# wz7in/CVPR2023-VLSAT

Hardware: AMD Instinct MI355X
Metric: scenes/sec (3RScan-shaped, N=40 obj x 256 pts) (higher is better)
Workload: dtype f32

## Files before the change

cvpr2023-vlsat_amd/build.py:

```python
from __future__ import annotations

import os
import shutil
import subprocess
import sys
from concurrent.futures import ThreadPoolExecutor

HERE = os.path.dirname(os.path.abspath(__file__))
CSRC = os.path.join(HERE, "csrc")
OBJ = os.path.join(HERE, "build")
LIB = os.path.join(HERE, "libvlsat_hip.so")
SOURCES = ["engine_weights.hip", "engine_plan.hip", "engine_forward.hip", "engine_api.hip", "gemm_f32.hip", "gemm_bf16_ring.hip", "gemm_bf16_p8.hip", "gemm_splitk.hip", "flash_attn_f32.hip", "flash_attn_bf16.hip", "pointnet.hip", "pointnet_bf16.hip", "edge_gate.hip", "edge_gate_bf16.hip", "edge_gate_heads.hip", "edge_gate_bf16_heads.hip", "small_ops.hip", "stn.hip", "eval_ranks.hip", "eval_recall.hip", "scene_graph.hip", "graph_decode.hip", "prep.hip", "proximity.hip", "label_transfer.hip", "segment_merge.hip", "scene_split.hip", "calibration.hip", "mesh_segment.hip", "cloud.hip", "voxel.hip", "objects.hip", "convex.hip", "comm.hip"]
FLAGS = ["--offload-arch=gfx950", "-O3", "-std=c++17", "-fPIC", "-ffp-contract=fast", "-Wall", "-Wno-unused-function", "-Wno-unused-value", "-Wno-unused-result"]
PER_SOURCE_FLAGS = {"proximity.hip": ["-ffp-contract=off"], "label_transfer.hip": ["-ffp-contract=off"],
                    "segment_merge.hip": ["-ffp-contract=off"], "scene_split.hip": ["-ffp-contract=off"],
                    "mesh_segment.hip": ["-ffp-contract=off"], "cloud.hip": ["-ffp-contract=off"],
                    "voxel.hip": ["-ffp-contract=off"], "objects.hip": ["-ffp-contract=off"],
                    "convex.hip": ["-ffp-contract=off"]}


def _hipcc() -> str:
    exe = shutil.which("hipcc") or "/opt/rocm/bin/hipcc"
    if not os.path.exists(exe):
        raise RuntimeError("hipcc not found; the HIP library cannot be built")
    return exe


def _newest_header() -> float:
    t = 0.0
    for d in (CSRC, os.path.join(os.path.dirname(HERE), "include")):
        for f in os.listdir(d):
            if f.endswith(".h"):
                t = max(t, os.path.getmtime(os.path.join(d, f)))
    return t


EXP_LIB = os.path.join(os.path.dirname(HERE), "tools", "bin", "libvlsat_hip_exp.so")


def build(force: bool = False, verbose: bool = False, experiments: bool = False) -> str:
    obj_dir = OBJ + "_exp" if experiments else OBJ
    lib = EXP_LIB if experiments else LIB
    flags = FLAGS + (["-DVLSAT_EXPERIMENTS"] if experiments else [])
    os.makedirs(obj_dir, exist_ok=True)
    os.makedirs(os.path.dirname(lib), exist_ok=True)
    hipcc = _hipcc()
    hdr_t = _newest_header()
    jobs = []
    objs = []
    for src in SOURCES:
        s = os.path.join(CSRC, src)
        o = os.path.join(obj_dir, src.replace(".hip", ".o"))
        objs.append(o)
        if force or not os.path.exists(o) or os.path.getmtime(o) < max(os.path.getmtime(s), hdr_t):
            jobs.append([hipcc, *flags, *PER_SOURCE_FLAGS.get(src, []), "-c", s, "-o", o])

    def run(cmd):
        if verbose:
            print(" ".join(cmd), flush=True)
        r = subprocess.run(cmd, capture_output=True, text=True)
        if r.returncode:
            raise RuntimeError(f"hipcc failed: {' '.join(cmd)}\n{r.stdout}\n{r.stderr}")
        return r.stderr

    with ThreadPoolExecutor(max_workers=min(8, max(1, len(jobs)))) as ex:
# ... 11 lines not shown
```

cvpr2023-vlsat_amd/csrc/edge_gate.hip:

```cpp
#include <cstdlib>
#include "gate_core.h"
#include "gate_agg.h"

namespace vlsat {

constexpr int GT_PITCH = 68;
constexpr int GT_PITCH3 = 132;

template <bool FUSED, bool TWIN = false>
__global__ __launch_bounds__(256, 2) void edge_gate_kernel(GateArgs pa, GateArgs pb) {
    const GateArgs& p = (TWIN && blockIdx.y != 0) ? pb : pa;
    __shared__ __attribute__((aligned(16))) float sW0[128 * GT_PITCH];
    __shared__ __attribute__((aligned(16))) float sW3[32 * GT_PITCH3];
    __shared__ __attribute__((aligned(16))) char sAgg[FUSED ? 4 * AG_WAVE_BYTES : 16];
    const int tid = threadIdx.x, lane = tid & 63, wave = tid >> 6;
    const int li = lane & 31, hi = lane >> 5;

    gate_stage_f32_rows<128, 128, 64, GT_PITCH, 256>(sW0, p.w0k, tid);
    gate_stage_f32_rows<32, 32, 128, GT_PITCH3, 256>(sW3, p.w3, tid);
    float b3f[16];
#pragma unroll
    for (int r = 0; r < 16; ++r) b3f[r] = p.b3[crow32(r, hi)];
    __syncthreads();

// ... 87 lines not shown
        if (valid) grow[m] = a;
    }
    if (!valid) return;
    const float inv = 1.f / sum;
    for (int m = 0; m < dox; ++m) {
        const float pr = grow[m] * inv;
        if (p.prob) p.prob[(size_t)e * (n_heads * dox) + m * n_heads + h] = pr;
        grow[m] = pr * vrow[m];
    }
}

int launch_gate_valu(const GateArgs& a, int n_heads, int dk, int dox, hipStream_t s) {
    if (dk < 1 || dk > 128 || dox < 1) return fail(-1, "edge_gate: unsupported head geometry");
    const long rows = (long)a.n_edges * n_heads;
    hipLaunchKernelGGL(edge_gate_generic_kernel, dim3((unsigned)((rows + 63) / 64)), dim3(64), 2 * dk * 64 * sizeof(float), s, a,
                       n_heads, dk, dox);
    VLSAT_LAUNCH_CHECK("edge_gate_generic");
    return 0;
}

int launch_gate_f32(const GateArgs& a, hipStream_t s, const GateArgs* twin) {
    const int n_groups = a.row_map ? 2 * ((a.n_edges + 31) / 32) : (a.n_edges + 15) / 16;
    const int cap = a.grid_cap > 0 ? a.grid_cap : (a.agg ? 512 : 768);
    const int grid = n_groups < cap ? n_groups : cap;
    if (twin) {
        if (a.agg) hipLaunchKernelGGL((edge_gate_kernel<true, true>), dim3(grid, 2), dim3(256), 0, s, a, *twin);
        else hipLaunchKernelGGL((edge_gate_kernel<false, true>), dim3(grid, 2), dim3(256), 0, s, a, *twin);
    } else if (a.agg) hipLaunchKernelGGL((edge_gate_kernel<true, false>), dim3(grid), dim3(256), 0, s, a, a);
    else hipLaunchKernelGGL((edge_gate_kernel<false, false>), dim3(grid), dim3(256), 0, s, a, a);
    VLSAT_LAUNCH_CHECK("edge_gate");
    return 0;
}

int launch_gate(GateKernel kernel, const GateArgs& a, int n_heads, int dk, int dox, int terms, int kproj_split, hipStream_t s,
                const GateArgs* twin) {
    if (a.n_edges <= 0) return 0;
    const GateChoice can = gate_choice(kernel);
    if (a.agg && !can.fuse_agg) return fail(-1, "edge_gate: this kernel does not implement the fused aggregation");
    if (twin && !can.twin) return fail(-1, "edge_gate: this kernel does not implement a twin launch");
    if (!a.row_map && !can.row_map0) return fail(-1, "edge_gate: this kernel has the 32-edges-per-wave row map only");
    if (twin && (twin->n_edges != a.n_edges || !twin->agg != !a.agg || twin->row_map != a.row_map || twin->use_edge != a.use_edge ||
                 !twin->prob != !a.prob || twin->grid_cap != a.grid_cap || twin->src != a.src || twin->dst != a.dst))
        return fail(-1, "edge_gate: a twin launch needs two problems on the same edge list with the same options");
    if (a.agg && (!a.row_map || a.prob || (a.ld_agg & 3))) return fail(-1, "edge_gate: the fused aggregation needs the 32-edges-per-wave row map and no prob tap");
    if (kernel != GATE_VALU && ((a.ld_node & 3) || (a.gq_off & 3) || (a.v_off & 3)))
        return fail(-1, "edge_gate: ld_node/gq_off/v_off must be multiples of 4");
    if (can.bits16()) {
        if (terms != 1 && terms != 3) return fail(-1, "edge_gate_bf16: terms must be 1 or 3");
        if (kproj_split >= 2 && terms != 1) return fail(-1, "edge_gate_bf16: half-row kproj needs terms = 1");
    }
    const bool shipped = n_heads == 8 && dk == 64 && dox == 32;
    switch (kernel) {
        case GATE_VALU: return launch_gate_valu(a, n_heads, dk, dox, s);
        case GATE_F32: case GATE_16:
            if (!shipped) return fail(-1, "edge_gate: the shipped kernels are built for 8 heads x (64, 32) only");
            return kernel == GATE_F32 ? launch_gate_f32(a, s, twin) : launch_gate_16(a, terms, kproj_split, s, twin);
        case GATE_F32_HEADS: case GATE_16_HEADS:
            if (!gate_heads_built(n_heads, dk, dox) || (kernel == GATE_16_HEADS && terms == 3 && dk == 128))
                return fail(-1, "edge_gate: head geometry / terms not built on the MFMA template");
            return kernel == GATE_F32_HEADS ? launch_gate_f32_heads(a, n_heads, dk, dox, s) : launch_gate_16_heads(a, n_heads, dk, dox, terms, kproj_split, s);
    }
    return fail(-1, "edge_gate: unknown kernel");
}

}
```

cvpr2023-vlsat_amd/csrc/engine.h:

```cpp
#pragma once
#include <cstddef>
#include <cstdint>

namespace vlsat {

struct EvalScratch {
    float *obj3, *obj2, *prob3, *prob2;
    float *rel3, *rel2;
    float* sorted;
    int32_t *or3, *or2;
    int32_t *rr3, *rr2, *tr3, *tr2;
    int32_t *cn3, *cn2;
};
inline size_t eval_scratch_edge_rows(size_t E) { return E > 0 ? E : 1; }
inline size_t eval_scratch_floats(size_t N, size_t E, size_t C, size_t R) { return 5 * N * C + 2 * eval_scratch_edge_rows(E) * R; }
inline size_t eval_scratch_ints(size_t N, size_t E, size_t R) { return 2 * N + (4 * R + 2) * eval_scratch_edge_rows(E); }
inline EvalScratch eval_scratch_carve(float* f, int32_t* i, size_t N, size_t E, size_t C, size_t R) {
    const size_t Es = eval_scratch_edge_rows(E);
    EvalScratch v;
    v.obj3 = f;                v.obj2 = v.obj3 + N * C;   v.prob3 = v.obj2 + N * C;  v.prob2 = v.prob3 + N * C;
    v.rel3 = v.prob2 + N * C;  v.rel2 = v.rel3 + Es * R;  v.sorted = v.rel2 + Es * R;
    v.or3 = i;                 v.or2 = v.or3 + N;
    v.rr3 = v.or2 + N;         v.rr2 = v.rr3 + Es * R;    v.tr3 = v.rr2 + Es * R;    v.tr2 = v.tr3 + Es * R;
    v.cn3 = v.tr2 + Es * R;    v.cn2 = v.cn3 + Es;
// ... 53 lines not shown
    int D = 512, A = 256, H = 8, C_pt = 768;
    std::map<std::string, std::vector<float>> host;
    bool finalized = false;
    std::vector<float*> dev_allocs;
    std::vector<std::pair<const float*, size_t>> gemm_w;
    float *pn_w1, *pn_b1, *pn_w2, *pn_b2, *pn_w3, *pn_b3;
    float *mlp_w, *mlp_b;
    float *re_w1cat, *re_b1cat;
    float *re3_w2, *re3_b2, *re3_w3, *re3_b3, *re2_w2, *re2_b2, *re2_w3, *re2_b3;
    float *ad_w1, *ad_b1, *ad_w2h, *ad_b2h;
    vlsat::DistBiasW db{};
    std::vector<vlsat::AttnW> self_attn, cross_attn, cross_rel;
    std::vector<vlsat::GcnW> gcn3, gcn2;
    vlsat::RelHeadW rel3{}, rel2{};
    vlsat::StnW stn_obj{}, stn_re3{}, stn_re2{};
    vlsat::TripletW trip{};
    float *obj3_w, *obj3_b, *obj2_w, *obj2_b;
    bool prof = false;
    struct Rec { int cls; hipEvent_t a, b; double flops; long kernels; };
    std::vector<Rec> recs;
    Rec open[3] = {};
    bool open_ok[3] = {false, false, false};
    hipEvent_t prof_base = nullptr;
    bool prof_base_set = false;
    int prof_dual = 1;
    std::vector<hipEvent_t> ev_pool;
    size_t ev_used = 0;
    double acc_ms[vlsat::PC_COUNT] = {0};
    int64_t acc_n[vlsat::PC_COUNT] = {0};
    double acc_fl[vlsat::PC_COUNT] = {0};
    int debug_stop = -1;
    int gemm_no_dma = 0, gate_grid = 0, gate_row_map = 1, gate_heads_mfma = 1, flash_heads_bf16 = 1, gate_heads_bf16 = 1;
    int pair_twins = 1;
    int pair_max_edges = 4096;
    int gather_f16 = -1;
    int outproj_f16 = -1;
    int gemm_k_rot = -1;
    int gemm_no_p8 = 0;
    int node_attn_split = 1024;
    long config_epoch = 0;
    int gemm_p8_part_min = 0;
    int gemm_splitk_max_tiles = 64;
    int gemm_splitk = 1;
    float* sk_ws[3] = {nullptr, nullptr, nullptr};
    unsigned* sk_cnt[3] = {nullptr, nullptr, nullptr};
    int flash_bq_big_min = 4096;
    int flash_qg = 0;
    int flash_bq_big = 1;
    int flash_dma = 1;
    int gate_fuse_agg = 1;
    int flash_ablate = 0;
    int flash_pv_terms = 3;
    int flash_exact = -1;
    int gemm_small_exact = -1;
    int pointnet_exact = -1;
    int edge_pairs = 1;
    vlsat::EdgePairs pairs{};
    int gemm_exact = -1;
    int ln_resid = 1;
    int half_fmt = 1;
    int split_fmt = 1;
    int pointnet_bf16 = 1, gate_bf16 = 1;
    int flash_bf16 = 1, flash_tr = 1;
    long gemm_launches = 0;
    int cur_N = -1;
    int prec = 0, prec_edge = 0, prec_node = 0;
    int half_f16 = 0;
    int prec_attn = 0;
    std::map<const float*, std::pair<uint16_t*, uint16_t*>> split;
    std::map<const float*, uint16_t*> f16w;
    struct F16sPlanes { uint16_t *hi, *lo; int k; };
    std::map<const float*, F16sPlanes> f16s;
    std::vector<vlsat::Arena> arena_pool;
    std::vector<vlsat::Arena> arena_trash;
    std::vector<vlsat::Staging> staging;
    std::vector<hipEvent_t> spare_ev;
};

struct vlsat_plan_s {
    vlsat_ctx* h = nullptr;
    int64_t N = 0, E = 0;
    int P = 0, S = 0, max_n = 0, is_fc = 0;
    std::vector<int32_t> node_ptr;
    std::vector<int64_t> edge_ptr;
    size_t ws_bytes = 0;
    vlsat::WsParams ws;
    char* arena = nullptr;
    size_t arena_bytes = 0;
    hipEvent_t uploaded = nullptr;
    bool upload_pending = false;
    hipEvent_t last_use = nullptr;
    bool used = false;
    int32_t *d_src, *d_dst, *d_rowptr, *d_order, *d_scene_ptr;
    int32_t* d_edge_ptr32 = nullptr;
    int max_e = 0;
    int64_t* d_bias_ptr;
    int4* d_tiles;
    int n_tiles = 0;
    int4* d_tiles_big = nullptr;
    int n_tiles_big = 0;
    int fa_parts = 1;
    int4* d_krange = nullptr;
    float *fa_opart = nullptr, *fa_m = nullptr, *fa_l = nullptr;
    double flash_flops = 0;
    float *F, *X3, *X2, *NP, *QKVn, *On, *T256, *T768, *rs, *bias;
    float *H1, *H2, *E3, *E2, *Hbig, *KP, *G, *Qe, *KVe, *Oe, *R1, *R2, *prob;
// ... 38 lines not shown
```

cvpr2023-vlsat_amd/csrc/engine_api.hip:

```cpp
#include <algorithm>
#include <climits>
#include <cstdint>
#include <cstring>
#include <vector>

#include "engine.h"

using namespace vlsat;

extern "C" {

const char* vlsat_last_error(void) { return last_error_cstr(); }

int vlsat_debug_stop_after(vlsat_handle h, int32_t stage) {
    if (!h) return fail(VLSAT_EINVAL, "null handle");
    h->debug_stop = stage;
    return 0;
}

int vlsat_debug_gemm_clock_probe(int64_t* buf) {
    gemm_set_clock_probe(reinterpret_cast<long long*>(buf));
    return 0;
}

int vlsat_set_edge_attention_scope(vlsat_handle h, int32_t scope) {
    if (!h) return fail(VLSAT_EINVAL, "null handle");
    if (scope != 0 && scope != 1) return fail(VLSAT_EINVAL, "edge attention scope: 0 (per scene) or 1 (whole batch)");
    h->edge_scope = scope;
    ++h->config_epoch;
    return 0;
}

int vlsat_debug_option(vlsat_handle h, const char* name, int32_t value) {
    if (!h || !name) return fail(VLSAT_EINVAL, "vlsat_debug_option: null argument");
    const std::string k(name);
    ++h->config_epoch;
    if (k == "dual_stream") h->dual_stream = value < 0 ? 0 : value;
    else if (k == "sched") h->sched = value < 0 ? -1 : value != 0;
    else if (k == "flash_split") h->fa_split = value != 0;
    else if (k == "gemm_dma") h->gemm_no_dma = value == 0;
    else if (k == "gemm_p8") h->gemm_no_p8 = value == 0;
    else if (k == "pair_twins") h->pair_twins = value != 0;
    else if (k == "pair_max_edges") h->pair_max_edges = value < 0 ? 0 : value;
    else if (k == "gather_f16") h->gather_f16 = value < 0 ? -1 : value != 0;
    else if (k == "outproj_f16") h->outproj_f16 = value < 0 ? -1 : value != 0;
    else if (k == "gemm_k_rot") h->gemm_k_rot = value < 0 ? -1 : value > 7 ? 7 : value;
    else if (k == "gate_row_map") h->gate_row_map = value != 0;
    else if (k == "prof_dual") h->prof_dual = value != 0;
    else if (k == "gate_heads_mfma") h->gate_heads_mfma = value < 0 ? 0 : value > 2 ? 2 : value;
    else if (k == "gemm_splitk") h->gemm_splitk = value != 0;
    else if (k == "gemm_p8_part_min") h->gemm_p8_part_min = value < 0 ? 0 : value;
    else if (k == "gemm_splitk_max_tiles") h->gemm_splitk_max_tiles = value < 0 ? 0 : value;
    else if (k == "split_fmt") h->split_fmt = value != 0;
    else if (k == "ln_resid") h->ln_resid = value != 0;
    else if (k == "gate_fuse_agg") h->gate_fuse_agg = value < 0 ? 0 : value > 2 ? 2 : value;
    else if (k == "flash_pv_terms") h->flash_pv_terms = value == 2 ? 2 : 3;
    else if (k == "flash_exact") h->flash_exact = value < 0 ? -1 : value != 0;
    else if (k == "edge_pairs") h->edge_pairs = value != 0;
    else if (k == "gemm_exact") h->gemm_exact = value < 0 ? -1 : value != 0;
    else if (k == "pointnet_exact") h->pointnet_exact = value < 0 ? -1 : value != 0;
    else if (k == "gemm_small_exact") h->gemm_small_exact = value < 0 ? -1 : value != 0;
    else if (k == "flash_bf16") h->flash_bf16 = value != 0;
    else if (k == "pointnet_bf16") h->pointnet_bf16 = value != 0;
    else if (k == "gate_bf16") h->gate_bf16 = value != 0;
    else if (k == "flash_tr") h->flash_tr = value != 0;
    else if (k == "flash_bq_big") h->flash_bq_big = value != 0;
    else if (k == "flash_qg") h->flash_qg = value < 0 || value > 2 ? 0 : value;
    else if (k == "flash_bq_big_min") h->flash_bq_big_min = value < 256 ? 256 : value;
#ifdef VLSAT_EXPERIMENTS
    else if (k == "gate_grid") h->gate_grid = value > 0 ? value : 0;
    else if (k == "gate_heads_bf16") h->gate_heads_bf16 = value != 0;
    else if (k == "flash_heads_bf16") h->flash_heads_bf16 = value != 0;
    else if (k == "node_attn_split") h->node_attn_split = value;
    else if (k == "half_fmt") h->half_fmt = value != 0;
    else if (k == "flash_dma") h->flash_dma = (value == 3 || value == 4) ? value : value != 0;
    else if (k == "flash_ablate") h->flash_ablate = value;
#else
    else if (k == "gate_grid" || k == "gate_heads_bf16" || k == "flash_heads_bf16" || k == "node_attn_split" || k == "half_fmt" ||
             k == "flash_dma" || k == "flash_ablate")
        return fail(VLSAT_EINVAL, "vlsat_debug_option: " + k + " is a lab switch of the experiments build (build.py --experiments)");
#endif
    else return fail(VLSAT_EINVAL, "vlsat_debug_option: unknown option " + k);
    return 0;
}

static int test_splitk_ws(GemmArgs& a) {
    static float* ws = nullptr;
    static unsigned* cnt = nullptr;
    if (!ws) {
        VLSAT_HIP_CHECK(hipMalloc(reinterpret_cast<void**>(&ws), SPLITK_WS_FLOATS * sizeof(float)));
        VLSAT_HIP_CHECK(hipMalloc(reinterpret_cast<void**>(&cnt), SPLITK_COUNTERS * sizeof(unsigned)));
        VLSAT_HIP_CHECK(hipMemset(cnt, 0, SPLITK_COUNTERS * sizeof(unsigned)));
    }
    a.sk_ws = ws; a.sk_ws_floats = SPLITK_WS_FLOATS; a.sk_counters = cnt; a.sk_n_counters = SPLITK_COUNTERS;
    return 0;
}

int vlsat_k_gemm(const float* A, int32_t lda, const float* W, int32_t ldw, float* C, int32_t ldc, int32_t M, int32_t N,
                 int32_t K, const float* bias, const float* rowscale, const float* resid, int32_t ldr, float resid_scale,
                 const float* g0, const int32_t* gi0, int32_t ldg0, const float* g1, const int32_t* gi1, int32_t ldg1,
                 int32_t relu_a, int32_t act, void* stream) {
    GemmArgs a;
    a.A = A; a.lda = lda; a.W = W; a.ldw = ldw; a.C = C; a.ldc = ldc; a.M = M; a.N = N; a.K = K;
    a.bias = bias; a.rowscale = rowscale; a.resid = resid; a.ldr = ldr; a.resid_scale = resid_scale;
    a.g0 = g0; a.gi0 = gi0; a.ldg0 = ldg0; a.g1 = g1; a.gi1 = gi1; a.ldg1 = ldg1; a.relu_a = relu_a & 1; a.act = act;
    if (relu_a & 2) a.prefetch = 0;
    if (relu_a & 4) RUN(test_splitk_ws(a));
    if (relu_a & 8) a.no_p8 = 1;
    if (kExperiments) {
        a.force_tile = (relu_a >> 4) & 7;
// ... 516 lines not shown
    hipStream_t s = static_cast<hipStream_t>(stream);
    const size_t Es = eval_scratch_edge_rows(E);
    const EvalScratch v = eval_scratch_carve(p->ev_f, p->ev_i, N, E, C, R);
    RUN(vlsat_forward(h, p, obj_points, obj_2d_feats, descriptor, v.obj3, do2d ? v.obj2 : nullptr, v.rel3, do2d ? v.rel2 : nullptr, stream));
    GraphDecodeWs ws;
    ws.ptr = v.or3;
    ws.cnt = v.rr3;
    ws.keys = reinterpret_cast<uint32_t*>(ws.cnt + Es);
    ws.preds = reinterpret_cast<uint8_t*>(ws.keys + Es * R);
    for (int br = 0; br < (do2d ? 2 : 1); ++br) {
        float* pr = br ? v.prob2 : v.prob3;
        float* rl = br ? v.rel2 : v.rel3;
        RUN(launch_softmax_rows(br ? v.obj2 : v.obj3, C, N, C, pr, 0, s));
        if (!h->d.multi_rel_outputs) RUN(launch_exp(rl, rl, (size_t)E * R, s));
        RUN(launch_graph_decode(pr, rl, edges_e2, nullptr, p->d_scene_ptr, thresholds, N, E, C, R, n_scenes, multi_label, score_mode,
                                n_labels, max_rel, ws, br ? labels_2d : labels_3d, br ? label_probs_2d : label_probs_3d,
                                br ? rels_2d : rels_3d, br ? scores_2d : scores_3d, br ? n_valid_2d : n_valid_3d,
                                br ? n_total_2d : n_total_3d, s));
    }
    VLSAT_HIP_CHECK(hipEventRecord(p->last_use, s));
    return 0;
}

namespace {
static int scene_tables(const int64_t* node_ptr, int n_scenes, int n_heads, std::vector<int32_t>& sp, std::vector<int64_t>& bp, int* max_n) {
    if (!node_ptr || n_scenes <= 0) return fail(VLSAT_EINVAL, "bad scene table");
    sp.resize(n_scenes + 1);
    bp.resize(n_scenes);
    int64_t off = 0;
    *max_n = 0;
    for (int s = 0; s <= n_scenes; ++s) {
        if (node_ptr[s] < 0 || node_ptr[s] > INT32_MAX || (s && node_ptr[s] < node_ptr[s - 1])) return fail(VLSAT_EINVAL, "scene table must be ascending int32 offsets");
        sp[s] = (int32_t)node_ptr[s];
        if (s < n_scenes) {
            const int64_t n = node_ptr[s + 1] - node_ptr[s];
            bp[s] = off;
            off += (int64_t)n_heads * n * n;
            if (n > *max_n) *max_n = (int)n;
        }
    }
    return 0;
}
}

int vlsat_k_edge_gate(const float* kproj, const float* node, int32_t ld_node, int32_t gq_off, int32_t v_off, const int32_t* src,
                      const int32_t* dst, const float* w0k, const float* w3, const float* b3, float* gated, float* prob,
                      int32_t n_edges, int32_t n_heads, int32_t dk, int32_t dox, int32_t use_edge, int32_t variant, void* stream) {
    if (!node || !src || !dst || !w3 || !b3 || !gated || (use_edge && (!kproj || !w0k))) return fail(VLSAT_EINVAL, "edge_gate: null argument");
    if (n_edges < 0 || n_heads <= 0 || dk <= 0 || dox <= 0) return fail(VLSAT_EINVAL, "edge_gate: bad geometry");
    hipStream_t s = static_cast<hipStream_t>(stream);
    GateArgs g{};
    g.kproj = kproj; g.node = node; g.ld_node = ld_node; g.gq_off = gq_off; g.v_off = v_off; g.src = src; g.dst = dst;
    g.w0k = w0k; g.w3 = w3; g.b3 = b3; g.gated = gated; g.prob = prob; g.n_edges = n_edges; g.use_edge = use_edge != 0;
    if (variant < 0 || variant > 4) return fail(VLSAT_EINVAL, "edge_gate: variant 0..4");
    const int terms = variant == 3 ? 3 : variant == 4 ? 1 : 0;
    const GateChoice gc = variant == 1 ? gate_choice(GATE_VALU) : gate_select(n_heads, dk, dox, terms, true, variant == 2 ? 2 : 1, true);
    if (variant == 2 && gc.kernel != GATE_F32_HEADS) return fail(VLSAT_EINVAL, "edge_gate: head geometry not built on the MFMA template");
    if (terms && !gc.bits16()) return fail(VLSAT_EINVAL, "edge_gate: head geometry / terms not built on the bf16 template");
    return launch_gate(gc.kernel, g, n_heads, dk, dox, terms, 0, s);
}

int vlsat_k_aggregate(const float* gated, int32_t n_ch, const int64_t* index_host, int64_t n_edges, int32_t n_nodes, int32_t aggr,
                      float* out, int32_t ldo, int32_t col0, void* stream) {
    if (!out || n_nodes < 0 || n_edges < 0 || n_ch <= 0 || (n_edges > 0 && (!gated || !index_host))) return fail(VLSAT_EINVAL, "aggregate: bad argument");
    if (aggr < 0 || aggr > 2) return fail(VLSAT_EINVAL, "aggregate: aggr 0 max | 1 add | 2 mean");
    if (n_edges > INT32_MAX) return fail(VLSAT_EINVAL, "aggregate: too many rows");
    std::vector<int32_t> rowptr(n_nodes + 1, 0), order((size_t)n_edges);
    for (int64_t e = 0; e < n_edges; ++e) {
        if (index_host[e] < 0 || index_host[e] >= n_nodes) return fail(VLSAT_EINVAL, "aggregate: index out of range");
        ++rowptr[index_host[e] + 1];
    }
    for (int n = 0; n < n_nodes; ++n) rowptr[n + 1] += rowptr[n];
    std::vector<int32_t> fill(rowptr.begin(), rowptr.end() - 1);
    for (int64_t e = 0; e < n_edges; ++e) order[fill[index_host[e]]++] = (int32_t)e;
    DevTable dr, dord;
    RUN(dr.put(rowptr.data(), rowptr.size() * sizeof(int32_t)));
    RUN(dord.put(order.data(), order.size() * sizeof(int32_t)));
    hipStream_t s = static_cast<hipStream_t>(stream);
    const int r = launch_aggregate(gated, n_ch, static_cast<const int32_t*>(dr.d), static_cast<const int32_t*>(dord.d), n_nodes, aggr, out, ldo, col0, s);
    hipStreamSynchronize(s);
    return r;
}

int vlsat_k_node_attn(const float* Q, int32_t ldq, const float* K, int32_t ldk, const float* V, int32_t ldv, float* O, int32_t ldo,
                      const float* bias, const int64_t* node_ptr_host, int32_t n_scenes, int32_t n_heads, float scale,
                      int32_t lanes_per_query, void* stream) {
    if (!Q || !K || !V || !O) return fail(VLSAT_EINVAL, "node_attn: null argument");
    if (n_heads <= 0 || 512 % n_heads) return fail(VLSAT_EINVAL, "node_attn: n_heads must divide 512");
    if (lanes_per_query != 0 && lanes_per_query != 1 && lanes_per_query != 16) return fail(VLSAT_EINVAL, "node_attn: lanes_per_query 0 (auto) | 1 | 16");
    std::vector<int32_t> sp;
    std::vector<int64_t> bp;
    int max_n = 0;
    RUN(scene_tables(node_ptr_host, n_scenes, n_heads, sp, bp, &max_n));
    DevTable dsp, dbp;
    RUN(dsp.put(sp.data(), sp.size() * sizeof(int32_t)));
    RUN(dbp.put(bp.data(), bp.size() * sizeof(int64_t)));
    hipStream_t s = static_cast<hipStream_t>(stream);
    const int split_below = lanes_per_query == 16 ? INT32_MAX : lanes_per_query == 1 ? 0 : 1024;
    const int r = launch_node_attn(Q, ldq, K, ldk, V, ldv, O, ldo, bias, static_cast<const int32_t*>(dsp.d), static_cast<const int64_t*>(dbp.d),
                                   n_scenes, max_n, n_heads, 512 / n_heads, scale, s, split_below);
    hipStreamSynchronize(s);
    return r;
}

int vlsat_k_dist_bias(const float* desc, int32_t ld_desc, const int64_t* node_ptr_host, int32_t n_scenes, int32_t n_heads,
                      const float* w0, const float* b0, const float* ln2_w, const float* ln2_b, const float* w3, const float* b3,
                      const float* ln5_w, const float* ln5_b, const float* w6, const float* b6, float* bias, void* stream) {
    if (!desc || !w0 || !b0 || !ln2_w || !ln2_b || !w3 || !b3 || !ln5_w || !ln5_b || !w6 || !b6 || !bias) return fail(VLSAT_EINVAL, "dist_bias: null argument");
    if (n_heads <= 0 || ld_desc < 3) return fail(VLSAT_EINVAL, "dist_bias: bad geometry");
// ... 91 lines not shown
```

cvpr2023-vlsat_amd/csrc/engine_forward.hip:

```cpp
#include <algorithm>
#include <cmath>
#include <cstring>

#include "engine.h"

using namespace vlsat;

static Scratch scratch_of(const vlsat_plan_s* p, int branch) {
    if (branch == 1 && p->dual)
        return {p->NP2, p->Hbig2, p->KP2, p->G2, p->T768b, p->Hbig2, p->Hbig2 + (size_t)std::max<int64_t>(p->E, 1) * 512, p->rs2, p->H2b};
    return {p->NP, p->Hbig, p->KP, p->G, p->T768, p->R1, p->R2, p->rs, p->H2};
}

namespace {

static int split_fmt(const vlsat_ctx* h) {
    const bool on = h->prec_edge != 0 && h->split_fmt && h->flash_bf16 && h->flash_tr && !h->gemm_no_dma && !h->d.feature_transform;
    if (!on) return 0;
    if (h->prec_edge == 3) return 1;
    return h->gate_bf16 && h->half_fmt ? 2 : 1;
}

static GateChoice gate_of(const vlsat_ctx* h) {
    return gate_select(h->H, h->D / h->H, h->A / h->H, h->prec_edge == 0 ? 0 : h->prec_edge == 3 ? 3 : 1, h->gate_bf16 != 0, h->gate_heads_mfma,
                       h->gate_heads_bf16 != 0);
}
static int gate_launch(vlsat_ctx* h, const GateChoice& gc, const GateArgs& g, hipStream_t s, const GateArgs* twin = nullptr) {
    const int S = gc.bits16() ? split_fmt(h) : 0;
    return launch_gate(gc.kernel, g, h->H, h->D / h->H, h->A / h->H, h->prec_edge == 3 ? 3 : 1, (S == 2 && h->half_f16) ? 3 : S, s, twin);
}
static bool gate_fuses_agg(const vlsat_ctx* h, const GateChoice& gc, const GateArgs& g) {
    return gc.fuse_agg && (h->gate_fuse_agg == 2 || (h->gate_fuse_agg == 1 && gc.bits16())) && h->d.gcn_aggr == 0 && !g.prob && h->debug_stop < 0 &&
           g.row_map && g.n_edges > 0;
}

hipEvent_t next_event(vlsat_ctx* h) {
    if (h->ev_used == h->ev_pool.size()) {
        hipEvent_t e;
        hipEventCreate(&e);
        h->ev_pool.push_back(e);
    }
    return h->ev_pool[h->ev_used++];
}
static inline int prof_lane(const vlsat_ctx* h, hipStream_t s) { return (h->side && s == h->side) ? 1 : (h->side2 && s == h->side2) ? 2 : 0; }
struct Scope {
    vlsat_ctx* h;
    hipStream_t s;
    int cls, w;
    double flops;
    long k0 = 0;
    Scope(vlsat_ctx* h_, hipStream_t s_, int cls_, double fl) : h(h_), s(s_), cls(cls_), w(prof_lane(h_, s_)), flops(fl) {
        k0 = h->gemm_launches;
        if (!h->prof) return;
        if (h->open_ok[w] && h->open[w].cls == cls) return;
        if (!h->prof_base_set) {
            if (!h->prof_base) hipEventCreate(&h->prof_base);
            hipEventRecord(h->prof_base, s);
            h->prof_base_set = true;
        }
        hipEvent_t e = next_event(h);
        hipEventRecord(e, s);
        if (h->open_ok[w]) { h->open[w].b = e; h->recs.push_back(h->open[w]); }
        h->open[w] = {cls, e, e, 0.0, 0};
        h->open_ok[w] = true;
    }
    ~Scope() {
        if (!h->prof) return;
        h->open[w].flops += flops;
        h->open[w].kernels += cls == PC_GEMM ? h->gemm_launches - k0 : 1;
    }
};
static void profile_close(vlsat_ctx* h, hipStream_t s) {
    const int w = prof_lane(h, s);
    if (!h->prof || !h->open_ok[w]) return;
    hipEvent_t e = next_event(h);
    hipEventRecord(e, s);
    h->open[w].b = e;
    h->recs.push_back(h->open[w]);
    h->open_ok[w] = false;
}

static int gemm_resolve(vlsat_ctx* h, int ws_lane, GemmArgs& a, int prec_override) {
    const bool edge_fmt = a.a_split || a.c_split || a.r_split;
    const int prec = prec_override >= 0 ? prec_override : (a.M == h->cur_N && !edge_fmt) ? h->prec_node : h->prec_edge;
    if (prec) {
// ... 727 lines not shown
```

cvpr2023-vlsat_amd/csrc/gate_core.h:

```cpp
#pragma once
#include "gemm_core.h"
#include "kernels.h"

namespace vlsat {

int launch_gate_valu(const GateArgs& a, int n_heads, int dk, int dox, hipStream_t s);
int launch_gate_f32(const GateArgs& a, hipStream_t s, const GateArgs* twin);
int launch_gate_f32_heads(const GateArgs& a, int n_heads, int dk, int dox, hipStream_t s);
int launch_gate_16(const GateArgs& a, int terms, int kproj_split, hipStream_t s, const GateArgs* twin);
int launch_gate_16_heads(const GateArgs& a, int n_heads, int dk, int dox, int terms, int kproj_split, hipStream_t s);

template <bool F16>
__device__ __forceinline__ bf16x4 gate_cv4(const f32x4& x) {
    if constexpr (F16) {
        typedef _Float16 f16x4_g __attribute__((ext_vector_type(4)));
        f32x4 y;
#pragma unroll
        for (int c = 0; c < 4; ++c) y[c] = __builtin_amdgcn_fmed3f(x[c], -65504.f, 65504.f);
        return __builtin_bit_cast(bf16x4, __builtin_convertvector(y, f16x4_g));
    } else {
        return __builtin_convertvector(x, bf16x4);
    }
}
__device__ __forceinline__ bf16x4 gate_lo4(const f32x4& x, const bf16x4& h) {
    return __builtin_convertvector(x - __builtin_convertvector(h, f32x4), bf16x4);
}
__device__ __forceinline__ bf16x8 gate_cat(const bf16x4& a, const bf16x4& b) { return __builtin_shufflevector(a, b, 0, 1, 2, 3, 4, 5, 6, 7); }
template <int PL, bool F16>
__device__ __forceinline__ void gate_split8(const f32x4& x0, const f32x4& x1, bf16x8& hi, bf16x8& lo) {
    const bf16x4 h0 = gate_cv4<F16>(x0), h1 = gate_cv4<F16>(x1);
    hi = gate_cat(h0, h1);
    lo = hi;
    if (PL == 2) lo = gate_cat(gate_lo4(x0, h0), gate_lo4(x1, h1));
}

template <int KS, int NK1>
__device__ __forceinline__ void gate_load_kproj(const float* krow, int col, bf16x8 (&zh)[NK1], bf16x8 (&zl)[NK1]) {
    typedef unsigned u32x4 __attribute__((ext_vector_type(4)));
    const float* zrow = krow + col;
#pragma unroll
    for (int ks = 0; ks < NK1; ++ks) {
        if (KS >= 2) {
            zh[ks] = *reinterpret_cast<const bf16x8*>(reinterpret_cast<const char*>(krow) + (col + 16 * ks) * 2);
            zl[ks] = zh[ks];
            continue;
        }
        const f32x4 x0 = *reinterpret_cast<const f32x4*>(zrow + 16 * ks), x1 = *reinterpret_cast<const f32x4*>(zrow + 16 * ks + 4);
        if (KS == 1) {
            const u32x4 a = __builtin_bit_cast(u32x4, x0), b = __builtin_bit_cast(u32x4, x1);
            u32x4 hh, ll;
            hh[0] = __builtin_amdgcn_perm(a[1], a[0], 0x07060302u); hh[1] = __builtin_amdgcn_perm(a[3], a[2], 0x07060302u);
            hh[2] = __builtin_amdgcn_perm(b[1], b[0], 0x07060302u); hh[3] = __builtin_amdgcn_perm(b[3], b[2], 0x07060302u);
            ll[0] = __builtin_amdgcn_perm(a[1], a[0], 0x05040100u); ll[1] = __builtin_amdgcn_perm(a[3], a[2], 0x05040100u);
            ll[2] = __builtin_amdgcn_perm(b[1], b[0], 0x05040100u); ll[3] = __builtin_amdgcn_perm(b[3], b[2], 0x05040100u);
            zh[ks] = __builtin_bit_cast(bf16x8, hh);
            zl[ks] = __builtin_bit_cast(bf16x8, ll);
        } else {
            gate_split8<2, false>(x0, x1, zh[ks], zl[ks]);
        }
    }
}

template <int ROWS, int N_VALID, int COLS, int PITCH, int NT>
// ... 124 lines not shown
```

cvpr2023-vlsat_amd/csrc/kernels.h:

```cpp
#pragma once
#include <hip/hip_runtime.h>
#include <stdint.h>

#include "flash_pick.h"
#include "gemm_plan.h"

namespace vlsat {

inline size_t align_up(size_t x, size_t a) { return (x + a - 1) & ~(a - 1); }

int launch_gemm(const GemmArgs& a, hipStream_t s);
int launch_gemm_pair(const GemmArgs& a, const GemmArgs& b, hipStream_t s);
int launch_gemm_splitk(const GemmArgs& a, const GemmPlan& p, hipStream_t s, const GemmArgs* twin = nullptr);
int launch_gemm_ring(const GemmArgs& a, const GemmPlan& p, hipStream_t s);
int launch_gemm_p8(const GemmArgs& a, const GemmPlan& p, hipStream_t s);
double gemm_flops(const GemmArgs& a);
void gemm_set_clock_probe(long long* buf);
int gemm_slots();

int launch_pointnet(const float* pts, int n_obj, int n_points, int cin, const float* w1, const float* b1,
                    const float* w2, const float* b2, const float* w3, const float* b3, int n_out,
                    float* out, hipStream_t s);

int launch_pointnet_bf16(const float* pts, int n_obj, int n_points, int cin, const float* w1, const float* b1,
// ... 18 lines not shown
                           const int4* tiles, int n_tiles, float scale_log2e, int terms, int use_tr, int io_split,
                           hipStream_t s, const FlashSplit* split = nullptr, int pv_terms = 3, int head_dim = 64);
int launch_flash_attn_f16x3(const float* Q, int ldq, const float* K, const float* V, int ldkv, float* O, int ldo,
                            const int4* tiles, int n_tiles, float scale_log2e, int use_tr, hipStream_t s,
                            const FlashSplit* split = nullptr, int head_dim = 64, int io = 0);

int launch_node_attn(const float* Q, int ldq, const float* K, int ldk, const float* V, int ldv,
                     float* O, int ldo, const float* bias, const int32_t* scene_ptr,
                     const int64_t* bias_ptr, int n_scenes, int max_n, int n_heads, int dk, float scale,
                     hipStream_t s, int split_below = 1024);
struct DistBiasW { const float *w0, *b0, *g2, *be2, *w3, *b3, *g5, *be5, *w6, *b6; };
int launch_dist_bias(const float* desc, int ld_desc, const int32_t* scene_ptr, const int64_t* bias_ptr,
                     int n_scenes, int max_n, int n_heads, DistBiasW w, float* bias, hipStream_t s);

int launch_edge_embed(const float* desc, const int32_t* src, const int32_t* dst, int n_edges,
                      const float* w1cat , const float* b1cat , float* h1, hipStream_t s);
int launch_desc_tail(const float* desc, int n_nodes, float* x, int ldx, int col0, hipStream_t s);
int launch_layernorm(float* x, int ld, int rows, int dim, const float* gamma, const float* beta, int relu,
                     hipStream_t s);
int launch_layernorm_to(const float* x, int ld, float* y, int ldy, int rows, int dim, const float* gamma, const float* beta,
                        int relu, int out_split, hipStream_t s, const float* resid = nullptr, int ldr = 0, int r_split = 0, int x_f16 = 0);
int launch_row_invnorm(const float* x, int ld, int rows, int dim, float scale, float* out, hipStream_t s, const float* x2 = nullptr, float* out2 = nullptr);

int launch_pts_conv1_rows(const float* pts, int n_obj, int P, int cin, const float* w1, const float* b1, float* rows,
                          hipStream_t s);
int launch_rowmax(const float* x, int ld, int n_obj, int P, int cols, float* out, int ldo, hipStream_t s);
int launch_apply_stn(const float* h, int ldh, const float* T, size_t rows, int P, float* out, int ldo, hipStream_t s);

struct GateArgs {
    const float* kproj;
    const float* node;
    int ld_node;
    int gq_off;
    int v_off;
    const int32_t* src;
    const int32_t* dst;
    const float* w0k;
    const float* w3;
    const float* b3;
    float* gated;
    float* prob;
    int n_edges;
    int use_edge = 1;
    int grid_cap = 0;
    float* agg = nullptr;
    int ld_agg = 0;
    int row_map = 1;
};
enum GateKernel {
    GATE_VALU,
    GATE_F32,
    GATE_F32_HEADS,
    GATE_16,
    GATE_16_HEADS
};
struct GateChoice {
    GateKernel kernel;
    bool fuse_agg;
    bool twin;
    bool row_map0;
    bool bits16() const { return kernel == GATE_16 || kernel == GATE_16_HEADS; }
};
inline GateChoice gate_choice(GateKernel k) {
    const bool shipped = k == GATE_F32 || k == GATE_16;
    return {k, shipped, shipped, shipped};
}
#define VLSAT_GATE_HEAD_GEOMETRIES(X) X(32, 8) X(32, 16) X(32, 32) X(64, 16) X(64, 32) X(64, 64) X(128, 32) X(128, 64) X(128, 128)
inline bool gate_heads_built(int n_heads, int dk, int dox) {
#define VLSAT_GH(DK, DOX) || (dk == DK && dox == DOX)
    return n_heads * dk == 512 && (false VLSAT_GATE_HEAD_GEOMETRIES(VLSAT_GH));
#undef VLSAT_GH
}
inline GateChoice gate_select(int n_heads, int dk, int dox, int terms, bool gate_bf16, int heads_mfma, bool heads_bf16) {
    const bool shipped = n_heads == 8 && dk == 64 && dox == 32 && heads_mfma != 2;
    const bool want16 = terms != 0 && gate_bf16;
    if (shipped) return gate_choice(want16 ? GATE_16 : GATE_F32);
    if (!heads_mfma || !gate_heads_built(n_heads, dk, dox)) return gate_choice(GATE_VALU);
    if (want16 && heads_bf16 && !(terms == 3 && dk == 128)) return gate_choice(GATE_16_HEADS);
    if (want16 && n_heads == 8 && dk == 64 && dox == 32) return gate_choice(GATE_16);
    return gate_choice(GATE_F32_HEADS);
}
int launch_gate(GateKernel kernel, const GateArgs& a, int n_heads, int dk, int dox, int terms, int kproj_split, hipStream_t s,
                const GateArgs* twin = nullptr);
int launch_agg_init(const int32_t* rowptr, int n_nodes, int n_ch, float* agg, int ld_agg, hipStream_t s, float* agg2 = nullptr);
int launch_zero_f32(float* p, size_t n, hipStream_t s);
int launch_copy_rows(float* dst, size_t dst_ld, const float* src, size_t src_ld, int cols, size_t rows, hipStream_t s);

int launch_aggregate(const float* gated, int n_ch, const int32_t* rowptr, const int32_t* order,
                     int n_nodes, int aggr, float* out, int ldo, int col0, hipStream_t s, const float* gated2 = nullptr, float* out2 = nullptr);

int launch_split_bf16(const float* w, size_t n, uint16_t* hi, uint16_t* lo, hipStream_t s);
int launch_to_f16(const float* w, size_t n, uint16_t* out, hipStream_t s);
int launch_split_f16s(const float* w, size_t n, uint16_t* hi, uint16_t* lo, unsigned* scratch2, hipStream_t s);

int launch_softmax_rows(const float* x, int ld, int rows, int cols, float* out, int log_out, hipStream_t s);
int launch_eval_ranks(const float* obj_logits, const float* obj_probs, const float* rel, const int64_t* gt_cls,
                      const int64_t* gt_rel, const int64_t* edges, int N, int E, int C, int R, int topk_obj,
                      int topk_rel, int topk_tri, float thr, int32_t* obj_rank, int32_t* rel_rank, int32_t* tri_rank,
                      int32_t* cnt, float* sorted_probs, hipStream_t s, bool rel_is_log);
inline int eval_ranks_sorted_k(int C, int topk_tri) { return C < topk_tri ? C : topk_tri; }

int launch_sort_probs(const float* probs, int N, int C, int K, float* sorted, hipStream_t s, int32_t* si = nullptr);
size_t eval_recallk_scratch_bytes(int64_t N, int64_t E, int C, int R, int n_scenes);
int launch_eval_recallk(const float* obj_probs, const float* rel, const int64_t* gt_cls, const int64_t* gt_rel, const int64_t* edges,
                        const int64_t* batch_ids, int N, int E, int C, int R, int n_scenes, int vmask, void* scratch,
                        long long* counts, hipStream_t s);

struct SceneGraphWs { float* sv; int32_t* si; int32_t* ptr; uint32_t* keys; uint32_t* packs; };
size_t scene_graph_scratch_bytes(int64_t N, int64_t E, int C, int R, int n_scenes, int each);
SceneGraphWs scene_graph_carve(void* scratch, int64_t N, int64_t E, int C, int R, int n_scenes, int each);
int scene_graph_check_args(int C, int R, int mode, int top_k, int each);
int launch_scene_graph_topk(const float* obj_probs, const float* rel, const int64_t* edges, const int64_t* batch_ids,
                            const int32_t* node_ptr, int N, int E, int C, int R, int n_scenes, int mode, int top_k, int each,
                            const SceneGraphWs& ws, int32_t* trip, float* score, int32_t* nvalid, hipStream_t s);
int launch_scene_edge_ptr(const int64_t* edges, const int64_t* batch_ids, const int32_t* node_ptr, int N, int E, int n_scenes, int32_t* ptr,
                          hipStream_t s);
int launch_exp(const float* x, float* out, size_t n, hipStream_t s);

struct GraphDecodeWs { int32_t* ptr; int32_t* cnt; uint32_t* keys; uint8_t* preds; };
size_t graph_decode_scratch_bytes(int64_t E, int R, int n_scenes);
GraphDecodeWs graph_decode_carve(void* scratch, int64_t E, int R, int n_scenes);
int graph_decode_check_args(int C, int R, int multi, int score_mode, int n_labels, int max_rel);
int launch_graph_decode(const float* obj_probs, const float* rel, const int64_t* edges, const int64_t* batch_ids, const int32_t* node_ptr,
                        const float* thr, int N, int E, int C, int R, int n_scenes, int multi, int score_mode, int n_labels, int max_rel,
                        const GraphDecodeWs& ws, int32_t* labels, float* label_probs, int32_t* rels, float* score, int32_t* nvalid,
                        int32_t* ntotal, hipStream_t s);
int launch_graph_decode_counts(const float* obj_probs, const float* rel, const int64_t* gt_cls, const int64_t* gt_rel, const float* thr,
                               int N, int E, int C, int R, int multi, unsigned long long* out, hipStream_t s);
// ... 60 lines not shown
```

Before: 4716.

## Add split-fp16 MFMA edge gate kernel and select it for exact f32 path

Adds a new edge-gate kernel that stages the weights as power-of-two-scaled fp16 hi/lo planes and computes the gate MLP with three fp16 MFMAs per step instead of f32 32x32x2 MFMAs. The kernel uses 8 waves per block, one edge-row unit per wave, and fuses max aggregation by default. It becomes the default when the edge precision is f32 (terms==0) unless gate_exact=1. The intent is to replace slow f32 matrix instructions with faster fp16 ones, trading exactness for a near-f32 split representation, with fp16 range clamping that could lose accuracy on large values.

```diff
diff --git a/cvpr2023-vlsat_amd/build.py b/cvpr2023-vlsat_amd/build.py
--- a/cvpr2023-vlsat_amd/build.py
+++ b/cvpr2023-vlsat_amd/build.py
@@ -10,7 +10,7 @@
 CSRC = os.path.join(HERE, "csrc")
 OBJ = os.path.join(HERE, "build")
 LIB = os.path.join(HERE, "libvlsat_hip.so")
-SOURCES = ["engine_weights.hip", "engine_plan.hip", "engine_forward.hip", "engine_api.hip", "gemm_f32.hip", "gemm_bf16_ring.hip", "gemm_bf16_p8.hip", "gemm_splitk.hip", "flash_attn_f32.hip", "flash_attn_bf16.hip", "pointnet.hip", "pointnet_bf16.hip", "edge_gate.hip", "edge_gate_bf16.hip", "edge_gate_heads.hip", "edge_gate_bf16_heads.hip", "small_ops.hip", "stn.hip", "eval_ranks.hip", "eval_recall.hip", "scene_graph.hip", "graph_decode.hip", "prep.hip", "proximity.hip", "label_transfer.hip", "segment_merge.hip", "scene_split.hip", "calibration.hip", "mesh_segment.hip", "cloud.hip", "voxel.hip", "objects.hip", "convex.hip", "comm.hip"]
+SOURCES = ["engine_weights.hip", "engine_plan.hip", "engine_forward.hip", "engine_api.hip", "gemm_f32.hip", "gemm_bf16_ring.hip", "gemm_bf16_p8.hip", "gemm_splitk.hip", "flash_attn_f32.hip", "flash_attn_bf16.hip", "pointnet.hip", "pointnet_bf16.hip", "edge_gate.hip", "edge_gate_bf16.hip", "edge_gate_f16s.hip", "edge_gate_heads.hip", "edge_gate_bf16_heads.hip", "small_ops.hip", "stn.hip", "eval_ranks.hip", "eval_recall.hip", "scene_graph.hip", "graph_decode.hip", "prep.hip", "proximity.hip", "label_transfer.hip", "segment_merge.hip", "scene_split.hip", "calibration.hip", "mesh_segment.hip", "cloud.hip", "voxel.hip", "objects.hip", "convex.hip", "comm.hip"]
 FLAGS = ["--offload-arch=gfx950", "-O3", "-std=c++17", "-fPIC", "-ffp-contract=fast", "-Wall", "-Wno-unused-function", "-Wno-unused-value", "-Wno-unused-result"]
 PER_SOURCE_FLAGS = {"proximity.hip": ["-ffp-contract=off"], "label_transfer.hip": ["-ffp-contract=off"],
                     "segment_merge.hip": ["-ffp-contract=off"], "scene_split.hip": ["-ffp-contract=off"],
diff --git a/cvpr2023-vlsat_amd/csrc/edge_gate.hip b/cvpr2023-vlsat_amd/csrc/edge_gate.hip
--- a/cvpr2023-vlsat_amd/csrc/edge_gate.hip
+++ b/cvpr2023-vlsat_amd/csrc/edge_gate.hip
@@ -163,8 +163,9 @@
     const bool shipped = n_heads == 8 && dk == 64 && dox == 32;
     switch (kernel) {
         case GATE_VALU: return launch_gate_valu(a, n_heads, dk, dox, s);
-        case GATE_F32: case GATE_16:
+        case GATE_F32: case GATE_16: case GATE_F16S:
             if (!shipped) return fail(-1, "edge_gate: the shipped kernels are built for 8 heads x (64, 32) only");
+            if (kernel == GATE_F16S) return launch_gate_f16s(a, s, twin);
             return kernel == GATE_F32 ? launch_gate_f32(a, s, twin) : launch_gate_16(a, terms, kproj_split, s, twin);
         case GATE_F32_HEADS: case GATE_16_HEADS:
             if (!gate_heads_built(n_heads, dk, dox) || (kernel == GATE_16_HEADS && terms == 3 && dk == 128))
diff --git a/cvpr2023-vlsat_amd/csrc/edge_gate_f16s.hip b/cvpr2023-vlsat_amd/csrc/edge_gate_f16s.hip
--- /dev/null
+++ b/cvpr2023-vlsat_amd/csrc/edge_gate_f16s.hip
@@ -0,0 +1,172 @@
+#include "gate_core.h"
+#include "gate_agg.h"
+#include "gemm_f16s_planes.h"
+
+namespace vlsat {
+
+namespace {
+
+constexpr int GF_P0 = 144;
+constexpr int GF_P3 = 264;
+constexpr int GF_NW = 8;
+constexpr int GF_NT = 64 * GF_NW;
+
+typedef float f32x8_g __attribute__((ext_vector_type(8)));
+typedef unsigned u32x4_g __attribute__((ext_vector_type(4)));
+typedef _Float16 f16x4_g __attribute__((ext_vector_type(4)));
+
+__device__ __forceinline__ void gf_split8(const f32x8_g& x, bf16x8& hi, bf16x8& lo) {
+    const u32x4_g h = __builtin_bit_cast(u32x4_g, __builtin_convertvector(x, f16x8));
+    u32x4_g l;
+#pragma unroll
+    for (int c = 0; c < 4; ++c) {
+        unsigned r;
+        asm("v_fma_mixlo_f16 %0, %1, -1.0, %2 op_sel_hi:[1,0,0]" : "=v"(r) : "v"(h[c]), "v"(x[2 * c]));
+        asm("v_fma_mixhi_f16 %0, %1, -1.0, %2 op_sel:[1,0,0] op_sel_hi:[1,0,0]" : "+v"(r) : "v"(h[c]), "v"(x[2 * c + 1]));
+        l[c] = r;
+    }
+    hi = __builtin_bit_cast(bf16x8, h);
+    lo = __builtin_bit_cast(bf16x8, l);
+}
+
+__device__ __forceinline__ unsigned gf_absmax(const float* w, int n4, int tid) {
+    unsigned m = 0;
+    for (int i = tid; i < n4; i += GF_NT) {
+        const u32x4_g v = *reinterpret_cast<const u32x4_g*>(w + 4 * i);
+#pragma unroll
+        for (int c = 0; c < 4; ++c) { const unsigned a = v[c] & 0x7fffffffu; m = a > m ? a : m; }
+    }
+    for (int o = 32; o > 0; o >>= 1) { const unsigned v = __shfl_xor(m, o); m = v > m ? v : m; }
+    return m;
+}
+template <int ROWS, int COLS, int PITCH>
+__device__ __forceinline__ void gf_stage_planes(char* sW, const float* w, float scale, int tid) {
+    for (int i = tid; i < ROWS * (COLS / 4); i += GF_NT) {
+        const int r = i / (COLS / 4), c4 = (i % (COLS / 4)) * 4;
+        f32x4 x = *reinterpret_cast<const f32x4*>(w + r * COLS + c4);
+#pragma unroll
+        for (int c = 0; c < 4; ++c) x[c] = __builtin_amdgcn_fmed3f(x[c] * scale, -65504.f, 65504.f);
+        const f16x4_g h = __builtin_convertvector(x, f16x4_g);
+        const f16x4_g l = __builtin_convertvector(x - __builtin_convertvector(h, f32x4), f16x4_g);
+        *reinterpret_cast<f16x4_g*>(sW + r * PITCH + c4 * 2) = h;
+        *reinterpret_cast<f16x4_g*>(sW + ROWS * PITCH + r * PITCH + c4 * 2) = l;
+    }
+}
+__device__ __forceinline__ f32x16 gf_mma3(const bf16x8& wh, const bf16x8& wl, const bf16x8& xh, const bf16x8& xl, const f32x16& acc) {
+    f32x16 c = mfma_h<true>(wh, xl, acc);
+    c = mfma_h<true>(wl, xh, c);
+    return mfma_h<true>(wh, xh, c);
+}
+
+template <bool TWIN>
+__global__ __launch_bounds__(GF_NT, 4) void edge_gate_f16s_kernel(GateArgs pa, GateArgs pb) {
+    const GateArgs& p = (TWIN && blockIdx.y != 0) ? pb : pa;
+    constexpr int W0B = 128 * GF_P0, W3B = 32 * GF_P3;
+    __shared__ __attribute__((aligned(16))) char smem[2 * (W0B + W3B) + GF_NW * AG_WAVE_BYTES];
+    __shared__ unsigned smax[2];
+    __shared__ __attribute__((aligned(16))) float sB3[32];
+    char* sW0 = smem;
+    char* sW3 = smem + 2 * W0B;
+    const int tid = threadIdx.x, lane = tid & 63, wave = tid >> 6;
+    const int li = lane & 31, hi = lane >> 5;
+
+    if (tid < 2) smax[tid] = 0;
+    __syncthreads();
+    {
+        const unsigned m0 = p.use_edge ? gf_absmax(p.w0k, 128 * 64 / 4, tid) : 0u, m3 = gf_absmax(p.w3, 32 * 128 / 4, tid);
+        if (lane == 0) { atomicMax(&smax[0], m0); atomicMax(&smax[1], m3); }
+    }
+    __syncthreads();
+    const int k0 = f16s_exponent(smax[0]), k3 = f16s_exponent(smax[1]);
+    if (p.use_edge) gf_stage_planes<128, 64, GF_P0>(sW0, p.w0k, f16s_pow2(k0), tid);
+    gf_stage_planes<32, 128, GF_P3>(sW3, p.w3, f16s_pow2(k3), tid);
+    const float inv0 = f16s_pow2(-k0), inv3 = f16s_pow2(-k3);
+    if (tid < 32) sB3[tid] = p.b3[tid] * f16s_pow2(k3);
+    __syncthreads();
+
+    const int n_units = (p.n_edges + 31) / 32;
+    const f32x16 zero = {0.f, 0.f, 0.f, 0.f, 0.f, 0.f, 0.f, 0.f, 0.f, 0.f, 0.f, 0.f, 0.f, 0.f, 0.f, 0.f};
+    for (int g = blockIdx.x; g < n_units; g += gridDim.x) {
+        asm volatile("" ::: "memory");
+        const int e_raw = p.row_map ? g * 32 + li : g * 32 + wave * 4 + (li >> 3);
+        const int h = p.row_map ? wave : li & 7;
+        const bool valid = e_raw < p.n_edges;
+        const int e = valid ? e_raw : p.n_edges - 1;
+        bf16x8 zh[4], zl[4];
+        if (p.use_edge) {
+            const float* zrow = p.kproj + (size_t)e * 512 + h * 64 + 8 * hi;
+#pragma unroll
+            for (int ks = 0; ks < 4; ++ks) {
+                const f32x4 x0 = *reinterpret_cast<const f32x4*>(zrow + 16 * ks), x1 = *reinterpret_cast<const f32x4*>(zrow + 16 * ks + 4);
+                f32x8_g x;
+#pragma unroll
+                for (int c = 0; c < 4; ++c) { x[c] = __builtin_amdgcn_fmed3f(x0[c], -65504.f, 65504.f); x[4 + c] = __builtin_amdgcn_fmed3f(x1[c], -65504.f, 65504.f); }
+                gf_split8(x, zh[ks], zl[ks]);
+            }
+        }
+        const int sn = p.src[e], dn = p.dst[e];
+        const float* gq = p.node + (size_t)sn * p.ld_node + p.gq_off + h * 128 + 4 * hi;
+        f32x16 lg[1];
+#pragma unroll
+        for (int r4 = 0; r4 < 4; ++r4) {
+            const f32x4 b = *reinterpret_cast<const f32x4*>(sB3 + 8 * r4 + 4 * hi);
+#pragma unroll
+            for (int c = 0; c < 4; ++c) lg[0][4 * r4 + c] = b[c];
+        }
+#pragma unroll
+        for (int to = 0; to < 4; ++to) {
+            f32x4 gqv[4];
+#pragma unroll
+            for (int r4 = 0; r4 < 4; ++r4) gqv[r4] = *reinterpret_cast<const f32x4*>(gq + to * 32 + 8 * r4);
+            float hid[16];
+            if (p.use_edge) {
+                const char* ap = sW0 + (to * 32 + li) * GF_P0 + 16 * hi;
+                f32x16 acc;
+#pragma unroll
+                for (int ks = 0; ks < 4; ++ks) {
+                    const bf16x8 wh = *reinterpret_cast<const bf16x8*>(ap + 32 * ks), wl = *reinterpret_cast<const bf16x8*>(ap + W0B + 32 * ks);
+                    acc = gf_mma3(wh, wl, zh[ks], zl[ks], ks == 0 ? zero : acc);
+                }
+#pragma unroll
+                for (int r = 0; r < 16; ++r) hid[r] = __builtin_amdgcn_fmed3f(__builtin_fmaf(acc[r], inv0, gqv[r >> 2][r & 3]), 0.f, 65504.f);
+            } else {
+#pragma unroll
+                for (int r = 0; r < 16; ++r) hid[r] = __builtin_amdgcn_fmed3f(gqv[r >> 2][r & 3], 0.f, 65504.f);
+            }
+#pragma unroll
+            for (int half = 0; half < 2; ++half) {
+                f32x8_g x;
+#pragma unroll
+                for (int c = 0; c < 8; ++c) x[c] = hid[8 * half + c];
+                bf16x8 hh, hl;
+                gf_split8(x, hh, hl);
+                const char* wp = sW3 + li * GF_P3 + (to * 32 + 16 * half + 4 * hi) * 2;
+                lg[0] = gf_mma3(gate_w3_frag(wp), gate_w3_frag(wp + W3B), hh, hl, lg[0]);
+            }
+        }
+#pragma unroll
+        for (int r = 0; r < 16; ++r) lg[0][r] *= inv3;
+        const float inv = gate_softmax<1, 32>(lg);
+        if (p.agg) {
+            gate_aggregate_max(smem + 2 * (W0B + W3B) + wave * AG_WAVE_BYTES, lg[0], inv, p.node + (size_t)dn * p.ld_node + p.v_off + h * 32 + 4 * hi,
+                               valid ? sn : -1, li, hi, lane, h, p.agg, p.ld_agg);
+        } else if (valid) {
+            gate_store<1, 32>(lg, inv, p.node + (size_t)dn * p.ld_node + p.v_off + h * 32 + 4 * hi, p.gated + (size_t)e * 256 + h * 32 + 4 * hi,
+                              p.prob, (size_t)e * 256, 8, h, hi);
+        }
+    }
+}
+
+}
+
+int launch_gate_f16s(const GateArgs& a, hipStream_t s, const GateArgs* twin) {
+    const int n_units = (a.n_edges + 31) / 32;
+    const int cap = a.grid_cap > 0 ? a.grid_cap : 512;
+    const int grid = n_units < cap ? n_units : cap;
+    if (twin) hipLaunchKernelGGL((edge_gate_f16s_kernel<true>), dim3(grid, 2), dim3(GF_NT), 0, s, a, *twin);
+    else hipLaunchKernelGGL((edge_gate_f16s_kernel<false>), dim3(grid), dim3(GF_NT), 0, s, a, a);
+    VLSAT_LAUNCH_CHECK("edge_gate_f16s");
+    return 0;
+}
+
+}
diff --git a/cvpr2023-vlsat_amd/csrc/engine.h b/cvpr2023-vlsat_amd/csrc/engine.h
--- a/cvpr2023-vlsat_amd/csrc/engine.h
+++ b/cvpr2023-vlsat_amd/csrc/engine.h
@@ -129,6 +129,7 @@
     int flash_ablate = 0;
     int flash_pv_terms = 3;
     int flash_exact = -1;
+    int gate_exact = -1;
     int gemm_small_exact = -1;
     int pointnet_exact = -1;
     int edge_pairs = 1;
diff --git a/cvpr2023-vlsat_amd/csrc/engine_api.hip b/cvpr2023-vlsat_amd/csrc/engine_api.hip
--- a/cvpr2023-vlsat_amd/csrc/engine_api.hip
+++ b/cvpr2023-vlsat_amd/csrc/engine_api.hip
@@ -56,6 +56,7 @@
     else if (k == "gate_fuse_agg") h->gate_fuse_agg = value < 0 ? 0 : value > 2 ? 2 : value;
     else if (k == "flash_pv_terms") h->flash_pv_terms = value == 2 ? 2 : 3;
     else if (k == "flash_exact") h->flash_exact = value < 0 ? -1 : value != 0;
+    else if (k == "gate_exact") h->gate_exact = value < 0 ? -1 : value != 0;
     else if (k == "edge_pairs") h->edge_pairs = value != 0;
     else if (k == "gemm_exact") h->gemm_exact = value < 0 ? -1 : value != 0;
     else if (k == "pointnet_exact") h->pointnet_exact = value < 0 ? -1 : value != 0;
@@ -678,9 +679,10 @@
     GateArgs g{};
     g.kproj = kproj; g.node = node; g.ld_node = ld_node; g.gq_off = gq_off; g.v_off = v_off; g.src = src; g.dst = dst;
     g.w0k = w0k; g.w3 = w3; g.b3 = b3; g.gated = gated; g.prob = prob; g.n_edges = n_edges; g.use_edge = use_edge != 0;
-    if (variant < 0 || variant > 4) return fail(VLSAT_EINVAL, "edge_gate: variant 0..4");
+    if (variant < 0 || variant > 5) return fail(VLSAT_EINVAL, "edge_gate: variant 0..5");
     const int terms = variant == 3 ? 3 : variant == 4 ? 1 : 0;
-    const GateChoice gc = variant == 1 ? gate_choice(GATE_VALU) : gate_select(n_heads, dk, dox, terms, true, variant == 2 ? 2 : 1, true);
+    const GateChoice gc = variant == 1 ? gate_choice(GATE_VALU) : gate_select(n_heads, dk, dox, terms, true, variant == 2 ? 2 : 1, true, variant == 5);
+    if (variant == 5 && gc.kernel != GATE_F16S) return fail(VLSAT_EINVAL, "edge_gate: the split-fp16 kernel is built for 8 heads x (64, 32) only");
     if (variant == 2 && gc.kernel != GATE_F32_HEADS) return fail(VLSAT_EINVAL, "edge_gate: head geometry not built on the MFMA template");
     if (terms && !gc.bits16()) return fail(VLSAT_EINVAL, "edge_gate: head geometry / terms not built on the bf16 template");
     return launch_gate(gc.kernel, g, n_heads, dk, dox, terms, 0, s);
diff --git a/cvpr2023-vlsat_amd/csrc/engine_forward.hip b/cvpr2023-vlsat_amd/csrc/engine_forward.hip
--- a/cvpr2023-vlsat_amd/csrc/engine_forward.hip
+++ b/cvpr2023-vlsat_amd/csrc/engine_forward.hip
@@ -21,16 +21,18 @@
     return h->gate_bf16 && h->half_fmt ? 2 : 1;
 }
 
+constexpr bool GATE_F16S_FUSES_AGG = true;
 static GateChoice gate_of(const vlsat_ctx* h) {
     return gate_select(h->H, h->D / h->H, h->A / h->H, h->prec_edge == 0 ? 0 : h->prec_edge == 3 ? 3 : 1, h->gate_bf16 != 0, h->gate_heads_mfma,
-                       h->gate_heads_bf16 != 0);
+                       h->gate_heads_bf16 != 0, h->gate_exact != 1);
 }
 static int gate_launch(vlsat_ctx* h, const GateChoice& gc, const GateArgs& g, hipStream_t s, const GateArgs* twin = nullptr) {
     const int S = gc.bits16() ? split_fmt(h) : 0;
     return launch_gate(gc.kernel, g, h->H, h->D / h->H, h->A / h->H, h->prec_edge == 3 ? 3 : 1, (S == 2 && h->half_f16) ? 3 : S, s, twin);
 }
 static bool gate_fuses_agg(const vlsat_ctx* h, const GateChoice& gc, const GateArgs& g) {
-    return gc.fuse_agg && (h->gate_fuse_agg == 2 || (h->gate_fuse_agg == 1 && gc.bits16())) && h->d.gcn_aggr == 0 && !g.prob && h->debug_stop < 0 &&
+    const bool by_default = gc.bits16() || (gc.kernel == GATE_F16S && GATE_F16S_FUSES_AGG);
+    return gc.fuse_agg && (h->gate_fuse_agg == 2 || (h->gate_fuse_agg == 1 && by_default)) && h->d.gcn_aggr == 0 && !g.prob && h->debug_stop < 0 &&
            g.row_map && g.n_edges > 0;
 }
 
diff --git a/cvpr2023-vlsat_amd/csrc/gate_core.h b/cvpr2023-vlsat_amd/csrc/gate_core.h
--- a/cvpr2023-vlsat_amd/csrc/gate_core.h
+++ b/cvpr2023-vlsat_amd/csrc/gate_core.h
@@ -9,6 +9,7 @@
 int launch_gate_f32_heads(const GateArgs& a, int n_heads, int dk, int dox, hipStream_t s);
 int launch_gate_16(const GateArgs& a, int terms, int kproj_split, hipStream_t s, const GateArgs* twin);
 int launch_gate_16_heads(const GateArgs& a, int n_heads, int dk, int dox, int terms, int kproj_split, hipStream_t s);
+int launch_gate_f16s(const GateArgs& a, hipStream_t s, const GateArgs* twin);
 
 template <bool F16>
 __device__ __forceinline__ bf16x4 gate_cv4(const f32x4& x) {
diff --git a/cvpr2023-vlsat_amd/csrc/kernels.h b/cvpr2023-vlsat_amd/csrc/kernels.h
--- a/cvpr2023-vlsat_amd/csrc/kernels.h
+++ b/cvpr2023-vlsat_amd/csrc/kernels.h
@@ -94,7 +94,8 @@
     GATE_F32,
     GATE_F32_HEADS,
     GATE_16,
-    GATE_16_HEADS
+    GATE_16_HEADS,
+    GATE_F16S
 };
 struct GateChoice {
     GateKernel kernel;
@@ -104,7 +105,7 @@
     bool bits16() const { return kernel == GATE_16 || kernel == GATE_16_HEADS; }
 };
 inline GateChoice gate_choice(GateKernel k) {
-    const bool shipped = k == GATE_F32 || k == GATE_16;
+    const bool shipped = k == GATE_F32 || k == GATE_16 || k == GATE_F16S;
     return {k, shipped, shipped, shipped};
 }
 #define VLSAT_GATE_HEAD_GEOMETRIES(X) X(32, 8) X(32, 16) X(32, 32) X(64, 16) X(64, 32) X(64, 64) X(128, 32) X(128, 64) X(128, 128)
@@ -113,9 +114,10 @@
     return n_heads * dk == 512 && (false VLSAT_GATE_HEAD_GEOMETRIES(VLSAT_GH));
 #undef VLSAT_GH
 }
-inline GateChoice gate_select(int n_heads, int dk, int dox, int terms, bool gate_bf16, int heads_mfma, bool heads_bf16) {
+inline GateChoice gate_select(int n_heads, int dk, int dox, int terms, bool gate_bf16, int heads_mfma, bool heads_bf16, bool f16s = false) {
     const bool shipped = n_heads == 8 && dk == 64 && dox == 32 && heads_mfma != 2;
     const bool want16 = terms != 0 && gate_bf16;
+    if (shipped && f16s && terms == 0) return gate_choice(GATE_F16S);
     if (shipped) return gate_choice(want16 ? GATE_16 : GATE_F32);
     if (!heads_mfma || !gate_heads_built(n_heads, dk, dox)) return gate_choice(GATE_VALU);
     if (want16 && heads_bf16 && !(terms == 3 && dk == 128)) return gate_choice(GATE_16_HEADS);
```

New measurement: 4712. Within noise of the previous version (-0.1%).
